# k2-fsa/Flow2GAN

Hardware: AMD Instinct MI355X
Metric: audio-seconds/sec (train step, G+D fwd/bwd) mel_24k_base (higher is better)
Workload: dtype f32 (fp32-class products on the bf16 matrix pipe for the long reductions and the direct MRD convs: every fp32 operand as three bf16 pieces = 24 significand bits, the six v_mfma_f32_32x32x16_bf16 products with i + j <= 2 per fp32 product, fp32 accumulate, error <= 2^-23 per product; short reductions ; 1 GPU; mel_24k_base GAN stage-2 train step: D-step + G-step, each on its own batch (MPD+MRD+FM+multi-scale mel), fwd+bwd+grad all-reduce, no optimizer (metric is fwd/bwd); per_gpu_batch=64, gan=gan_multi_scale_mel_recon, parallelism=dp1, optimizer=none

## Files before the change

### flow2gan_amd/csrc/conv32x6.hip

```cpp
#include <stdlib.h>

#include "common.h"


namespace {

typedef float f32x16 __attribute__((ext_vector_type(16)));
typedef float f32x4 __attribute__((ext_vector_type(4)));
typedef __bf16 bf16x8 __attribute__((ext_vector_type(8)));
typedef unsigned int u32x2 __attribute__((ext_vector_type(2)));
typedef unsigned int u32x4 __attribute__((ext_vector_type(4)));

constexpr int C = 32, KH = 3, KW = 9, NTAP = KH * KW;
constexpr int PB = 208;
constexpr int TG = 4;
constexpr int WBB = C * PB;
constexpr int WCH = C * 12;

__device__ __attribute__((aligned(16))) float c6_zero[4] = {0.f, 0.f, 0.f, 0.f};

__device__ __forceinline__ void split3(const f32x4 v, u32x2& p0, u32x2& p1, u32x2& p2) {
  unsigned a0, a1, a2, b0, b1, b2;
  f2g_split3_pair(v.x, v.y, a0, a1, a2);
  f2g_split3_pair(v.z, v.w, b0, b1, b2);
  p0 = u32x2{a0, b0};
  p1 = u32x2{a1, b1};
  p2 = u32x2{a2, b2};
}

__device__ __forceinline__ void store_px3(unsigned char* p, const f32x4 v) {
  u32x2 p0, p1, p2;
  split3(v, p0, p1, p2);
  *reinterpret_cast<u32x2*>(p) = p0;
  *reinterpret_cast<u32x2*>(p + 64) = p1;
  *reinterpret_cast<u32x2*>(p + 128) = p2;
}

struct frag6 {
  bf16x8 v[2][3];
};
__device__ __forceinline__ void ld6(frag6& f, const unsigned char* p) {
#pragma unroll
  for (int ks = 0; ks < 2; ++ks)
#pragma unroll
    for (int q = 0; q < 3; ++q) f.v[ks][q] = *reinterpret_cast<const bf16x8*>(p + q * 64 + ks * 32);
}
__device__ __forceinline__ void mm6(const frag6& a, const frag6& b, f32x16& acc0, f32x16& acc1) {
#define F2G_X6_PAIR(I, J)                                                               \
  acc0 = __builtin_amdgcn_mfma_f32_32x32x16_bf16(a.v[0][I], b.v[0][J], acc0, 0, 0, 0);   \
  acc1 = __builtin_amdgcn_mfma_f32_32x32x16_bf16(a.v[1][I], b.v[1][J], acc1, 0, 0, 0);
  F2G_X6_PAIR(2, 0) F2G_X6_PAIR(1, 1) F2G_X6_PAIR(0, 2) F2G_X6_PAIR(1, 0) F2G_X6_PAIR(0, 1) F2G_X6_PAIR(0, 0)
#undef F2G_X6_PAIR
}
__device__ __forceinline__ void tap6(const unsigned char* Ab, const unsigned char* Bb, f32x16& acc0, f32x16& acc1) {
  frag6 a, b;
  ld6(a, Ab);
  ld6(b, Bb);
  mm6(a, b, acc0, acc1);
}

template <int D>
__device__ __forceinline__ int div_small(int x) {
  static_assert(D == 39 || D == 23 || D == 20 || D == 12, "magic constants below");
  return (x * (D == 39 ? 1681 : D == 23 ? 2850 : D == 20 ? 3277 : 5462)) >> 16;
}

template <int TW_>
__device__ __forceinline__ void px_of_row(int pg, int r, int& ph, int& pw) {
  if (TW_ == 16) {
    ph = 2 * pg + (r >> 4);
    pw = (r + 12 * (r >> 4)) & 15;
  } else {
    const int p = pg * 32 + r;
    ph = p / TW_;
    pw = p % TW_;
  }
}

struct wplan {
  int src[3];
  int dst[3];
  int u[3];
};

template <int TH_, int TW_>
__global__ __launch_bounds__(512, 1) void conv32_s2_fwd6_kernel(const f2g_conv32_desc d, int tiles_w,
                                                               int tiles_h, int ntiles) {
  constexpr int IHv = TH_ + KH - 1, IWv = TW_ + (KW - 1) / 2, XW = 2 * IWv - 1;
  constexpr int SUBB = IHv * IWv * PB + 64;
  constexpr int NCHK = (IHv * XW * (C / 4) + 511) / 512;
  constexpr int NG = (NTAP + TG - 1) / TG + 1;
  static_assert(NG % 2 == 0, "the weight double buffer must come back to buffer 0 at a tile's end");
  static_assert(TH_ * TW_ == 128, "a block owns 128 output pixels");
  extern __shared__ __attribute__((aligned(16))) unsigned char smb[];
  unsigned char* At = smb;
  unsigned char* Bt = smb + 2 * SUBB;
  float* red = reinterpret_cast<float*>(Bt + 2 * TG * WBB);
  const int tid = threadIdx.x, lane = tid & 63, wave = tid >> 6;
  const int li = lane & 31, hh = lane >> 5;
  const int pg = wave & 3, half = wave >> 2;
  const int c4 = tid & 7;
  const int px0 = tid >> 3;
  auto tile_pos = [&](int tile, int& sq, int& h0, int& w0) {
    const int tw = tile % tiles_w, rest = tile / tiles_w;
    const int th = rest % tiles_h;
    sq = rest / tiles_h;
    h0 = th * TH_;
    w0 = tw * TW_;
  };
  auto load_patch = [&](int tile, f32x4 (&pf)[NCHK]) {
    int sq, h0, w0;
    tile_pos(tile, sq, h0, w0);
    const int x0 = 2 * w0 - (KW - 1) / 2;
    const float* org = d.x + (long long)sq * d.x_seq + (long long)(h0 - 1) * d.x_line + (long long)x0 * C + c4 * 4;
#pragma unroll
    for (int q = 0; q < NCHK; ++q) {
      const int px = px0 + 64 * q;
      const int r = div_small<XW>(px), xr = px - r * XW;
      const int h = h0 - 1 + r, x = x0 + xr;
      const bool ok = px < IHv * XW && h >= 0 && h < d.H && x >= 0 && x < d.Win;
      pf[q] = *reinterpret_cast<const f32x4*>(ok ? org + (long long)r * d.x_line + xr * C : c6_zero);
    }
  };
  auto store_patch = [&](const f32x4 (&pf)[NCHK]) {
// ... 53 lines not shown
    f32x16 acc0, acc1;
#pragma unroll
    for (int e = 0; e < 16; ++e) { acc0[e] = 0.f; acc1[e] = 0.f; }
#pragma unroll
    for (int g = 0; g < NG; ++g) {
      load_w(g + 1 < NG ? g + 1 : 0, wn);
      const int buf = g & 1;
#pragma unroll
      for (int u2 = 0; u2 < 2; ++u2) {
        const int t0 = g * TG + u2, t1 = g * TG + 2 + u2;
        if (t0 < NTAP && (half ? t1 : t0) < NTAP)
          tap6(Ap + (half ? F2G_C6_AOFF(t1) : F2G_C6_AOFF(t0)), Bp + (buf * TG + half * 2 + u2) * WBB, acc0, acc1);
      }
      store_w(buf ^ 1, wn);
      __syncthreads();
    }
#undef F2G_C6_AOFF
#pragma unroll
    for (int e = 0; e < 16; ++e) acc0[e] += acc1[e];
    if (half == 1) {
#pragma unroll
      for (int e = 0; e < 16; ++e) red[(pg * 16 + e) * 64 + lane] = acc0[e];
    }
    if (more) store_patch(pf);
    __syncthreads();
    if (half == 0) {
      int sq, h0, w0;
      tile_pos(tile, sq, h0, w0);
      float* ys = d.y + (long long)sq * d.y_seq;
      float* turn = red + pg * (16 * 64);
      float v[16];
#pragma unroll
      for (int e = 0; e < 16; ++e) {
        v[e] = acc0[e] + red[(pg * 16 + e) * 64 + lane] + bias;
        if (d.lrelu_slope != 0.f) v[e] = v[e] > 0.f ? v[e] : d.lrelu_slope * v[e];
      }
      __builtin_amdgcn_wave_barrier();
#pragma unroll
      for (int e = 0; e < 16; ++e) turn[((e & 3) + 8 * (e >> 2) + 4 * hh) * 32 + li] = v[e];
      __builtin_amdgcn_wave_barrier();
#pragma unroll
      for (int j = 0; j < 4; ++j) {
        int qh, qw;
        px_of_row<TW_>(pg, (lane >> 3) + 8 * j, qh, qw);
        const int oh = h0 + qh, ow = w0 + qw;
        const f32x4 u = *reinterpret_cast<const f32x4*>(turn + ((lane >> 3) + 8 * j) * 32 + 4 * (lane & 7));
        if (oh < d.H && ow < d.Wout)
          *reinterpret_cast<f32x4*>(ys + (long long)oh * d.y_line + (long long)ow * C + 4 * (lane & 7)) = u;
      }
    }
  }
}

template <int TH_, int TW_>
__global__ __launch_bounds__(512, 1) void conv32_s2_dgrad6_kernel(const f2g_conv32_desc d, int tiles_w,
                                                                 int tiles_h, int ntiles) {
  constexpr int IHv = TH_ + KH - 1, GWv = TW_ + 4;
  constexpr int NCHK = (IHv * GWv * (C / 4) + 511) / 512;
  constexpr int NG = 8;
  static_assert(TH_ * TW_ == 128, "a block owns 128 positions of each column parity");
  extern __shared__ __attribute__((aligned(16))) unsigned char smb[];
  unsigned char* At = smb;
  unsigned char* Bt = smb + IHv * GWv * PB;
  float* turn = reinterpret_cast<float*>(Bt + 2 * TG * WBB) + (threadIdx.x >> 6) * (32 * 32);
  const int tid = threadIdx.x, lane = tid & 63, wave = tid >> 6;
  const int li = lane & 31, hh = lane >> 5;
  const int pg = wave & 3, E = wave >> 2;
  const int c4 = tid & 7;
  const int NU = E ? 4 : 5, NT = KH * NU;
  const int Wp = (d.Win + 1 - E) / 2;
  const int px0 = tid >> 3;
  auto tile_pos = [&](int tile, int& sq, int& h0, int& m0) {
    const int tw = tile % tiles_w, rest = tile / tiles_w;
    const int th = rest % tiles_h;
    sq = rest / tiles_h;
    h0 = th * TH_;
    m0 = tw * TW_;
  };
  auto load_patch = [&](int tile, f32x4 (&pf)[NCHK]) {
    int sq, h0, m0;
    tile_pos(tile, sq, h0, m0);
    const float* org = d.x + (long long)sq * d.x_seq + (long long)(h0 - 1) * d.x_line + (long long)(m0 - 2) * C + c4 * 4;
#pragma unroll
    for (int q = 0; q < NCHK; ++q) {
      const int px = px0 + 64 * q;
      const int r = div_small<GWv>(px), xc = px - r * GWv;
      const int h = h0 - 1 + r, c = m0 - 2 + xc;
      const bool ok = px < IHv * GWv && h >= 0 && h < d.H && c >= 0 && c < d.Wout;
      pf[q] = *reinterpret_cast<const f32x4*>(ok ? org + (long long)r * d.x_line + xc * C : c6_zero);
    }
  };
  auto store_patch = [&](const f32x4 (&pf)[NCHK]) {
#pragma unroll
    for (int q = 0; q < NCHK; ++q) {
      const int px = px0 + 64 * q;
      if (px < IHv * GWv) store_px3(At + px * PB + c4 * 8, pf[q]);
    }
  };
  const unsigned char* wimg = reinterpret_cast<const unsigned char*>(d.w);
  int wsrc[3], wdst[3], wslot[3];
#pragma unroll
  for (int k = 0; k < 3; ++k) {
    const int c = tid + 512 * k;
    const int u = c / WCH, rem = c - u * WCH;
    const int row = rem / 12, part = rem - row * 12;
    wslot[k] = u;
    wsrc[k] = row * 192 + part * 16;
    wdst[k] = u * WBB + row * PB + part * 16;
  }
  auto load_w = [&](int g, u32x4 (&wn)[3]) {
#pragma unroll
    for (int k = 0; k < 3; ++k) {
      const int e = wslot[k] >> 1, nu = e ? 4 : 5, nt = KH * nu;
      int ti = 2 * g + (wslot[k] & 1);
      ti = ti < nt ? ti : nt - 1;
      const int dh = e ? ti >> 2 : (ti * 13) >> 6;
      const int tile_w = dh * KW + e + 2 * (ti - dh * nu);
      wn[k] = *reinterpret_cast<const u32x4*>(wimg + (long long)tile_w * (C * 192) + wsrc[k]);
    }
  };
  auto store_w = [&](int buf, const u32x4 (&wn)[3]) {
#pragma unroll
    for (int k = 0; k < 3; ++k) *reinterpret_cast<u32x4*>(Bt + buf * (TG * WBB) + wdst[k]) = wn[k];
  };
  int ph, pw;
  px_of_row<TW_>(pg, li, ph, pw);
  const unsigned char* Ap = At + ((ph + 2) * GWv + pw + 4) * PB + hh * 16;
  const unsigned char* Bp = Bt + (E * 2) * WBB + li * PB + hh * 16;
  const bool msk = d.mask_src != nullptr, fm = d.fm_ref != nullptr;
  const float fmw = fm ? d.fm_w * (d.fm_wdev ? d.fm_wdev[0] : 1.f) : 0.f;
  float cs[4] = {0.f, 0.f, 0.f, 0.f};

  int tile = blockIdx.x;
  if (tile >= ntiles) return;
  u32x4 wn[3];
  {
    f32x4 pf[NCHK];
    load_patch(tile, pf);
    load_w(0, wn);
    store_patch(pf);
    store_w(0, wn);
  }
  __syncthreads();
  for (; tile < ntiles; tile += gridDim.x) {
    const int nxt = tile + gridDim.x;
    const bool more = nxt < ntiles;
    f32x4 pf[NCHK];
    load_patch(more ? nxt : tile, pf);
    int sq, h0, m0;
    tile_pos(tile, sq, h0, m0);
    long long ioff[4];
    f32x4 my[4];
#pragma unroll
    for (int j = 0; j < 4; ++j) {
      int qh, qw;
      px_of_row<TW_>(pg, (lane >> 3) + 8 * j, qh, qw);
      const int oh = h0 + qh, om = m0 + qw;
      ioff[j] = (oh < d.H && om < Wp)
                    ? (long long)sq * d.y_seq + (long long)oh * d.y_line + (long long)(2 * om + E) * C + 4 * (lane & 7)
                    : -1;
      if (msk && !fm) my[j] = *reinterpret_cast<const f32x4*>(d.mask_src + (ioff[j] >= 0 ? ioff[j] : 0));
    }
    f32x16 acc0, acc1;
#pragma unroll
    for (int e = 0; e < 16; ++e) { acc0[e] = 0.f; acc1[e] = 0.f; }
#define F2G_C6_GOFF(TI) ((E ? ((TI) / 4) * GWv + (TI) % 4 : ((TI) / 5) * GWv + (TI) % 5) * PB)
#pragma unroll
    for (int g = 0; g < NG; ++g) {
      load_w(g + 1 < NG ? g + 1 : 0, wn);
      const int buf = g & 1;
#pragma unroll
      for (int u2 = 0; u2 < 2; ++u2)
        if (2 * g + u2 < NT) tap6(Ap - F2G_C6_GOFF(2 * g + u2), Bp + (buf * TG + u2) * WBB, acc0, acc1);
      store_w(buf ^ 1, wn);
      __syncthreads();
    }
#undef F2G_C6_GOFF
#pragma unroll
    for (int q = 0; q < 16; ++q) turn[((q & 3) + 8 * (q >> 2) + 4 * hh) * 32 + li] = acc0[q] + acc1[q];
    __builtin_amdgcn_wave_barrier();
    auto item = [&](int j) {
      return *reinterpret_cast<const f32x4*>(turn + ((lane >> 3) + 8 * j) * 32 + 4 * (lane & 7));
    };
    if (!msk) {
#pragma unroll
      for (int j = 0; j < 4; ++j) {
        const f32x4 u = item(j);
        if (ioff[j] < 0) continue;
        cs[0] += u.x, cs[1] += u.y, cs[2] += u.z, cs[3] += u.w;
        *reinterpret_cast<f32x4*>(d.y + ioff[j]) = u;
      }
    } else if (!fm) {
#pragma unroll
      for (int j = 0; j < 4; ++j) {
        const f32x4 u = item(j);
        if (ioff[j] < 0) continue;
        f32x4 v;
        v.x = u.x * (my[j].x > 0.f ? 1.f : d.mask_slope);
        v.y = u.y * (my[j].y > 0.f ? 1.f : d.mask_slope);
        v.z = u.z * (my[j].z > 0.f ? 1.f : d.mask_slope);
        v.w = u.w * (my[j].w > 0.f ? 1.f : d.mask_slope);
        cs[0] += v.x, cs[1] += v.y, cs[2] += v.z, cs[3] += v.w;
        *reinterpret_cast<f32x4*>(d.y + ioff[j]) = v;
      }
    } else {
      f32x4 yv[4], fv[4];
#pragma unroll
      for (int j = 0; j < 4; ++j) {
        const long long o = ioff[j] >= 0 ? ioff[j] : 0;
        yv[j] = *reinterpret_cast<const f32x4*>(d.mask_src + o);
        fv[j] = *reinterpret_cast<const f32x4*>(d.fm_ref + o);
      }
#pragma unroll
      for (int j = 0; j < 4; ++j) {
        const f32x4 u = item(j);
        if (ioff[j] < 0) continue;
        float v[4] = {u.x, u.y, u.z, u.w};
        const float y[4] = {yv[j].x, yv[j].y, yv[j].z, yv[j].w}, f[4] = {fv[j].x, fv[j].y, fv[j].z, fv[j].w};
#pragma unroll
        for (int e = 0; e < 4; ++e) {
          const float dl = y[e] - f[e];
          v[e] += fmw * (dl > 0.f ? 1.f : (dl < 0.f ? -1.f : 0.f));
          v[e] *= y[e] > 0.f ? 1.f : d.mask_slope;
          cs[e] += v[e];
        }
        *reinterpret_cast<f32x4*>(d.y + ioff[j]) = f32x4{v[0], v[1], v[2], v[3]};
      }
    }
    __builtin_amdgcn_wave_barrier();
    if (more) store_patch(pf);
    __syncthreads();
  }
  if (d.colsum) {
#pragma unroll
    for (int e = 0; e < 4; ++e) {
      float v = cs[e];
      v += __shfl_xor(v, 8);
      v += __shfl_xor(v, 16);
      v += __shfl_xor(v, 32);
      if (lane < 8) atomicAdd(d.colsum + 4 * lane + e, v);
    }
  }
}

template <int TH_, int TW_>
__global__ __launch_bounds__(512, 1) void conv32_s2_dgrad6m_kernel(const f2g_conv32_desc d, int tiles_w,
                                                                 int tiles_h, int ntiles) {
  constexpr int IHv = TH_ + KH - 1, GWv = TW_ + 4;
  constexpr int NCHK = (IHv * GWv * (C / 4) + 511) / 512;
  constexpr int NG = 8;
  static_assert(TH_ * TW_ == 128, "a block owns 128 positions of each column parity");
  extern __shared__ __attribute__((aligned(16))) unsigned char smb[];
  unsigned char* At = smb;
  unsigned char* Bt = smb + IHv * GWv * PB;
  const int tid = threadIdx.x, lane = tid & 63, wave = tid >> 6;
  const int li = lane & 31, hh = lane >> 5;
  const int pg = wave & 3, E = wave >> 2;
  const int c4 = tid & 7;
  const int NU = E ? 4 : 5, NT = KH * NU;
  const int Wp = (d.Win + 1 - E) / 2;
  const int px0 = tid >> 3;
  auto tile_pos = [&](int tile, int& sq, int& h0, int& m0) {
    const int tw = tile % tiles_w, rest = tile / tiles_w;
    const int th = rest % tiles_h;
    sq = rest / tiles_h;
    h0 = th * TH_;
    m0 = tw * TW_;
  };
  auto load_patch = [&](int tile, f32x4 (&pf)[NCHK]) {
    int sq, h0, m0;
    tile_pos(tile, sq, h0, m0);
    const float* org = d.x + (long long)sq * d.x_seq + (long long)(h0 - 1) * d.x_line + (long long)(m0 - 2) * C + c4 * 4;
#pragma unroll
    for (int q = 0; q < NCHK; ++q) {
      const int px = px0 + 64 * q;
      const int r = div_small<GWv>(px), xc = px - r * GWv;
      const int h = h0 - 1 + r, c = m0 - 2 + xc;
      const bool ok = px < IHv * GWv && h >= 0 && h < d.H && c >= 0 && c < d.Wout;
      pf[q] = *reinterpret_cast<const f32x4*>(ok ? org + (long long)r * d.x_line + xc * C : c6_zero);
    }
  };
  auto store_patch = [&](const f32x4 (&pf)[NCHK]) {
#pragma unroll
    for (int q = 0; q < NCHK; ++q) {
      const int px = px0 + 64 * q;
      if (px < IHv * GWv) store_px3(At + px * PB + c4 * 8, pf[q]);
    }
  };
  const unsigned char* wimg = reinterpret_cast<const unsigned char*>(d.w);
  int wsrc[3], wdst[3], wslot[3];
#pragma unroll
  for (int k = 0; k < 3; ++k) {
    const int c = tid + 512 * k;
    const int u = c / WCH, rem = c - u * WCH;
    const int row = rem / 12, part = rem - row * 12;
    wslot[k] = u;
    wsrc[k] = row * 192 + part * 16;
    wdst[k] = u * WBB + row * PB + part * 16;
  }
  auto load_w = [&](int g, u32x4 (&wn)[3]) {
#pragma unroll
    for (int k = 0; k < 3; ++k) {
      const int e = wslot[k] >> 1, nu = e ? 4 : 5, nt = KH * nu;
      int ti = 2 * g + (wslot[k] & 1);
      ti = ti < nt ? ti : nt - 1;
      const int dh = e ? ti >> 2 : (ti * 13) >> 6;
      const int tile_w = dh * KW + e + 2 * (ti - dh * nu);
      wn[k] = *reinterpret_cast<const u32x4*>(wimg + (long long)tile_w * (C * 192) + wsrc[k]);
    }
  };
  auto store_w = [&](int buf, const u32x4 (&wn)[3]) {
#pragma unroll
    for (int k = 0; k < 3; ++k) *reinterpret_cast<u32x4*>(Bt + buf * (TG * WBB) + wdst[k]) = wn[k];
  };
  int ph, pw;
  px_of_row<TW_>(pg, li, ph, pw);
  const unsigned char* Ap = At + ((ph + 2) * GWv + pw + 4) * PB + hh * 16;
  const unsigned char* Bp = Bt + (E * 2) * WBB + li * PB + hh * 16;
  const bool msk = d.mask_src != nullptr, fm = d.fm_ref != nullptr;
  const float fmw = fm ? d.fm_w * (d.fm_wdev ? d.fm_wdev[0] : 1.f) : 0.f;
  float cs = 0.f;

  int tile = blockIdx.x;
  if (tile >= ntiles) return;
  u32x4 wn[3];
  {
    f32x4 pf[NCHK];
    load_patch(tile, pf);
    load_w(0, wn);
    store_patch(pf);
    store_w(0, wn);
  }
  __syncthreads();
  for (; tile < ntiles; tile += gridDim.x) {
    const int nxt = tile + gridDim.x;
    const bool more = nxt < ntiles;
    f32x4 pf[NCHK];
    load_patch(more ? nxt : tile, pf);
    int sq, h0, m0;
    tile_pos(tile, sq, h0, m0);
    float my[16];
    if (msk && !fm) {
#pragma unroll
      for (int q = 0; q < 16; ++q) {
        int qh, qw;
        px_of_row<TW_>(pg, (q & 3) + 8 * (q >> 2) + 4 * hh, qh, qw);
        const int oh = h0 + qh, om = m0 + qw;
        const long long off = (long long)sq * d.y_seq + (long long)oh * d.y_line + (long long)(2 * om + E) * C + li;
        my[q] = (oh < d.H && om < Wp) ? d.mask_src[off] : 1.f;
      }
    }
    f32x16 acc0, acc1;
#pragma unroll
    for (int e = 0; e < 16; ++e) { acc0[e] = 0.f; acc1[e] = 0.f; }
#define F2G_C6_GOFF(TI) ((E ? ((TI) / 4) * GWv + (TI) % 4 : ((TI) / 5) * GWv + (TI) % 5) * PB)
#pragma unroll
    for (int g = 0; g < NG; ++g) {
      load_w(g + 1 < NG ? g + 1 : 0, wn);
      const int buf = g & 1;
#pragma unroll
      for (int u2 = 0; u2 < 2; ++u2)
        if (2 * g + u2 < NT) tap6(Ap - F2G_C6_GOFF(2 * g + u2), Bp + (buf * TG + u2) * WBB, acc0, acc1);
      store_w(buf ^ 1, wn);
      __syncthreads();
    }
#undef F2G_C6_GOFF
#pragma unroll
    for (int q = 0; q < 16; ++q) {
      int qh, qw;
      px_of_row<TW_>(pg, (q & 3) + 8 * (q >> 2) + 4 * hh, qh, qw);
      const int oh = h0 + qh, om = m0 + qw;
      if (oh < d.H && om < Wp) {
        const long long off = (long long)sq * d.y_seq + (long long)oh * d.y_line + (long long)(2 * om + E) * C + li;
        float v = acc0[q] + acc1[q];
        if (msk) {
          const float y = fm ? d.mask_src[off] : my[q];
          if (fm) {
            const float dl = y - d.fm_ref[off];
            v += fmw * (dl > 0.f ? 1.f : (dl < 0.f ? -1.f : 0.f));
          }
          v *= y > 0.f ? 1.f : d.mask_slope;
        }
        cs += v;
        d.y[off] = v;
      }
    }
    if (more) store_patch(pf);
    __syncthreads();
  }
  if (d.colsum) {
    cs += __shfl_xor(cs, 32);
    if (hh == 0) atomicAdd(d.colsum + li, cs);
  }
}

typedef short s16x4 __attribute__((ext_vector_type(4)));
constexpr int GPL = 128 * 64;
constexpr int GCH = 128 * (C / 4) / 512;

__device__ __forceinline__ bf16x8 tr_pix8(const unsigned char* p) {
  typedef s16x4 __attribute__((address_space(3))) * lds_p;
  const s16x4 a = __builtin_amdgcn_ds_read_tr16_b64_v4i16((lds_p)(p));
  const s16x4 b = __builtin_amdgcn_ds_read_tr16_b64_v4i16((lds_p)(p + 4 * 64));
  return __builtin_bit_cast(bf16x8, __builtin_shufflevector(a, b, 0, 1, 2, 3, 4, 5, 6, 7));
}

template <int TH, int TW>
__global__ __launch_bounds__(512, 1) void conv32_s2_wgrad6_kernel(const f2g_conv32_desc d, float* gw,
                                                                  int tiles_h, int tiles_w,
                                                                  int tiles_per_block) {
  constexpr int IH = TH + KH - 1, IW = TW + (KW - 1) / 2, XW = 2 * IW - 1;
  constexpr int XPAR = IH * IW * 64 + 64;
  constexpr int XPL = 2 * XPAR;
  constexpr int XCH = (IH * XW * (C / 4) + 511) / 512;
  constexpr int KR = 16 / TW;
  constexpr int NK = TH / KR;
  static_assert(TH * TW == 128 && NK == 8 && XCH <= NK && GCH <= NK, "tile shapes");
  extern __shared__ __attribute__((aligned(16))) unsigned char smb[];
  unsigned char* Xp = smb;
  unsigned char* Gp = smb + 3 * XPL;
  const int tid = threadIdx.x, lane = tid & 63, wave = tid >> 6;
  const int li = lane & 31, hh = lane >> 5;
  const int ntiles = d.S * tiles_h * tiles_w;
  f32x16 acc[6];
#pragma unroll
  for (int a = 0; a < 6; ++a)
#pragma unroll
    for (int e = 0; e < 16; ++e) acc[a][e] = 0.f;
  const int g4 = lane >> 4, i16 = lane & 15;
  const int kpix = (g4 >> 1) * 8 + (i16 >> 2);
  const int kpat = TW == 16 ? kpix : (g4 >> 1) * IW + (i16 >> 2);
  const int chb = (g4 & 1) * 32 + (i16 & 3) * 8;
  int xo[3], xs[3];
#pragma unroll
  for (int a = 0; a < 3; ++a) {
    int t = wave + 8 * a;
    int dh = t / KW, j = t - dh * KW;
    xo[a] = (j & 1) * XPAR + (dh * IW + (j >> 1) + kpat) * 64 + chb;
    t = 24 + a;
    dh = t / KW;
    j = t - dh * KW;
    xs[a] = (j & 1) * XPAR + (dh * IW + (j >> 1) + kpat) * 64 + chb;
  }
  const int go = kpix * 64 + chb;
  const int c4 = tid & 7, px0 = tid >> 3;
// ... 321 lines not shown
    for (int q = 0; q < NQ; ++q) {
      const int px = (tid + 512 * q) >> 3;
      u32x2 pk[3];
      if (xrow[q] > -(1 << 21)) {
        split3(px_[q], pk[0], pk[1], pk[2]);
#pragma unroll
        for (int pc = 0; pc < 3; ++pc) *reinterpret_cast<u32x2*>(Xp + pc * W33_XPL + (px + 1) * 64 + c4 * 8) = pk[pc];
      }
      if (grow[q] > -(1 << 21)) {
        split3(pg_[q], pk[0], pk[1], pk[2]);
#pragma unroll
        for (int pc = 0; pc < 3; ++pc) *reinterpret_cast<u32x2*>(Gp + pc * W33_GPL + px * 64 + c4 * 8) = pk[pc];
      }
    }
    __syncthreads();
    for (int ks = wave; ks < nks; ks += 8) {
      bf16x8 a[3];
#pragma unroll
      for (int q = 0; q < 3; ++q) a[q] = tr_pix8(Gp + q * W33_GPL + ks * (16 * 64) + go);
#pragma unroll
      for (int t = 0; t < T33; ++t) {
        bf16x8 b[3];
#pragma unroll
        for (int q = 0; q < 3; ++q) b[q] = tr_pix8(Xp + q * W33_XPL + ks * (16 * 64) + xo[t]);
        mfma6(a, b, acc[t]);
      }
    }
    __syncthreads();
  }
  float* red = reinterpret_cast<float*>(smb);
#pragma unroll
  for (int t = 0; t < T33; ++t) {
    __syncthreads();
#pragma unroll
    for (int e = 0; e < 16; ++e) red[(wave * 16 + e) * 64 + lane] = acc[t][e];
    __syncthreads();
    if (wave == (t & 7)) {
#pragma unroll
      for (int e = 0; e < 16; ++e) {
        float v = 0.f;
#pragma unroll
        for (int w8 = 0; w8 < 8; ++w8) v += red[(w8 * 16 + e) * 64 + lane];
        const int co = (e & 3) + 8 * (e >> 2) + 4 * hh;
        atomicAdd(gw + co * (T33 * C) + t * C + li, v);
      }
    }
  }
}

template <int TH_, int TW_>
constexpr size_t fwd6_smem() {
  return (size_t)2 * ((TH_ + 2) * (TW_ + 4) * PB + 64) + 2 * TG * WBB + 4 * 16 * 64 * sizeof(float);
}
template <int TH_, int TW_>
constexpr size_t dgrad6_smem() {
  return (size_t)(TH_ + 2) * (TW_ + 4) * PB + 2 * TG * WBB + 8 * 32 * 32 * sizeof(float);
}

}

int f2g_conv32_fwd6_launch(const f2g_conv32_desc* d, hipStream_t st) {
  auto waste = [&](int th, int tw) {
    return (long long)((d->H + th - 1) / th * th) * ((d->Wout + tw - 1) / tw * tw);
  };
  const bool tall = waste(16, 8) < waste(8, 16);
  const int th = tall ? 16 : 8, tw = tall ? 8 : 16;
  const int tiles_h = (d->H + th - 1) / th, tiles_w = (d->Wout + tw - 1) / tw;
  const long long nt = (long long)tiles_h * tiles_w * d->S;
  if (nt >= (1ll << 30) || d->x_line >= (1ll << 24)) return F2G_EINVAL;
  static bool attr = false;
  if (!attr) {
    (void)hipFuncSetAttribute(reinterpret_cast<const void*>(conv32_s2_fwd6_kernel<8, 16>),
                              hipFuncAttributeMaxDynamicSharedMemorySize, (int)(fwd6_smem<8, 16>()));
    (void)hipFuncSetAttribute(reinterpret_cast<const void*>(conv32_s2_fwd6_kernel<16, 8>),
                              hipFuncAttributeMaxDynamicSharedMemorySize, (int)(fwd6_smem<16, 8>()));
    attr = true;
  }
  const int grid = (int)(nt < 256 ? nt : 256);
  if (tall)
    hipLaunchKernelGGL((conv32_s2_fwd6_kernel<16, 8>), dim3(grid), dim3(512), (fwd6_smem<16, 8>()), st, *d,
                       tiles_w, tiles_h, (int)nt);
  else
    hipLaunchKernelGGL((conv32_s2_fwd6_kernel<8, 16>), dim3(grid), dim3(512), (fwd6_smem<8, 16>()), st, *d,
                       tiles_w, tiles_h, (int)nt);
  return f2g_check_launch();
}

int f2g_conv32_dgrad6_launch(const f2g_conv32_desc* d, hipStream_t st) {
  const int Wp0 = (d->Win + 1) / 2;
  auto waste = [&](int th, int tw) {
    return (long long)((d->H + th - 1) / th * th) * ((Wp0 + tw - 1) / tw * tw);
  };
  const bool tall = waste(16, 8) < waste(8, 16);
  const int th = tall ? 16 : 8, tw = tall ? 8 : 16;
  const int tiles_h = (d->H + th - 1) / th, tiles_w = (Wp0 + tw - 1) / tw;
  const long long nt = (long long)tiles_h * tiles_w * d->S;
  if (nt >= (1ll << 30) || d->x_line >= (1ll << 24)) return F2G_EINVAL;
  static bool attr = false;
  if (!attr) {
    (void)hipFuncSetAttribute(reinterpret_cast<const void*>(conv32_s2_dgrad6_kernel<8, 16>),
                              hipFuncAttributeMaxDynamicSharedMemorySize, (int)(dgrad6_smem<8, 16>()));
    (void)hipFuncSetAttribute(reinterpret_cast<const void*>(conv32_s2_dgrad6_kernel<16, 8>),
                              hipFuncAttributeMaxDynamicSharedMemorySize, (int)(dgrad6_smem<16, 8>()));
    attr = true;
  }
  const int grid = (int)(nt < 256 ? nt : 256);
  if (d->mask_src) {
    static bool attrm = false;
    if (!attrm) {
      (void)hipFuncSetAttribute(reinterpret_cast<const void*>(conv32_s2_dgrad6m_kernel<8, 16>),
                                hipFuncAttributeMaxDynamicSharedMemorySize, (int)(dgrad6_smem<8, 16>()));
      (void)hipFuncSetAttribute(reinterpret_cast<const void*>(conv32_s2_dgrad6m_kernel<16, 8>),
                                hipFuncAttributeMaxDynamicSharedMemorySize, (int)(dgrad6_smem<16, 8>()));
      attrm = true;
    }
    if (tall)
      hipLaunchKernelGGL((conv32_s2_dgrad6m_kernel<16, 8>), dim3(grid), dim3(512), (dgrad6_smem<16, 8>()), st, *d,
                         tiles_w, tiles_h, (int)nt);
    else
      hipLaunchKernelGGL((conv32_s2_dgrad6m_kernel<8, 16>), dim3(grid), dim3(512), (dgrad6_smem<8, 16>()), st, *d,
                         tiles_w, tiles_h, (int)nt);
    return f2g_check_launch();
  }
  if (tall)
    hipLaunchKernelGGL((conv32_s2_dgrad6_kernel<16, 8>), dim3(grid), dim3(512), (dgrad6_smem<16, 8>()), st, *d,
                       tiles_w, tiles_h, (int)nt);
  else
    hipLaunchKernelGGL((conv32_s2_dgrad6_kernel<8, 16>), dim3(grid), dim3(512), (dgrad6_smem<8, 16>()), st, *d,
                       tiles_w, tiles_h, (int)nt);
  return f2g_check_launch();
}

int f2g_conv32_wgrad6_launch(const f2g_conv32_desc* d, float* gw, hipStream_t st) {
  auto waste = [&](int th, int tw) {
    return (long long)((d->H + th - 1) / th * th) * ((d->Wout + tw - 1) / tw * tw);
  };
  const bool tall = waste(16, 8) < waste(8, 16);
  const int th = tall ? 16 : 8, tw = tall ? 8 : 16;
  const int tiles_h = (d->H + th - 1) / th, tiles_w = (d->Wout + tw - 1) / tw;
  const long long nt = (long long)d->S * tiles_h * tiles_w;
  if (nt >= (1ll << 30) || d->x_line >= (1ll << 24)) return F2G_EINVAL;
  int per = (int)((nt + 255) / 256);
  if (per < 1) per = 1;
  constexpr size_t sm8 = (size_t)3 * 2 * ((8 + 2) * (16 + 4) * 64 + 64) + 3 * GPL;
  constexpr size_t sm16 = (size_t)3 * 2 * ((16 + 2) * (8 + 4) * 64 + 64) + 3 * GPL;
  static_assert(sm8 >= (size_t)8 * 16 * 64 * 4 && sm16 >= (size_t)8 * 16 * 64 * 4,
                "the flush reuses the planes as its reduction buffer");
  static bool attr = false;
  if (!attr) {
    (void)hipFuncSetAttribute(reinterpret_cast<const void*>(conv32_s2_wgrad6_kernel<8, 16>),
                              hipFuncAttributeMaxDynamicSharedMemorySize, (int)sm8);
    (void)hipFuncSetAttribute(reinterpret_cast<const void*>(conv32_s2_wgrad6_kernel<16, 8>),
                              hipFuncAttributeMaxDynamicSharedMemorySize, (int)sm16);
    attr = true;
  }
  const unsigned grid = (unsigned)((nt + per - 1) / per);
  if (tall)
    hipLaunchKernelGGL((conv32_s2_wgrad6_kernel<16, 8>), dim3(grid), dim3(512), sm16, st, *d, gw, tiles_h, tiles_w, per);
  else
    hipLaunchKernelGGL((conv32_s2_wgrad6_kernel<8, 16>), dim3(grid), dim3(512), sm8, st, *d, gw, tiles_h, tiles_w, per);
  return f2g_check_launch();
}

extern "C" int f2g_conv33_fwd(const f2g_conv32_desc* d, f2g_stream_t stream) {
  if (!d || !d->x || !d->w || !d->y || d->precision != 3 || d->Win != d->Wout || d->fm_ref) return F2G_EINVAL;
  if ((((uintptr_t)d->x) & 15) || (((uintptr_t)d->w) & 15) || (d->x_line & 3) || (d->x_seq & 3)) return F2G_EINVAL;
  if (d->S <= 0 || d->H <= 0 || d->Win <= 0) return F2G_OK;
  const int W = d->Win;
  if (W > 112 || d->x_line >= (1ll << 24)) return F2G_EINVAL;
  if (d->y_line < (long long)W * C || (d->y != d->x && d->y_seq < (long long)d->H * d->y_line)) return F2G_EINVAL;
  if ((d->y_line & 3) || (d->y_seq & 3) || (((uintptr_t)d->y) & 15)) return F2G_EINVAL;
  if (d->mask_src && (d->lrelu_slope != 0.f || d->bias || (((uintptr_t)d->mask_src) & 15))) {
    f2g_set_error("f2g_conv33_fwd: mask_src (data-gradient role) excludes bias / lrelu_slope (forward role)");
    return F2G_EINVAL;
  }
  int R = 256 / W;
  if (R > d->H) R = d->H;
  while (R > 1 && (R + 2) * (W + 2) > P33) --R;
  if (R < 1 || (R + 2) * (W + 2) > P33) return F2G_EINVAL;
  const int tiles_h = (d->H + R - 1) / R;
  const long long nt = (long long)tiles_h * d->S;
  if (nt >= (1ll << 30)) return F2G_EINVAL;
// ... 44 lines not shown
```

Before: 804.1 audio-s/s.

## Restructure stride-2 conv dgrad so each wave computes both output parities

The dgrad kernel is reorganised so every wave owns both even and odd output columns of a 256-position tile, instead of splitting waves by parity. Each A fragment loaded from LDS now feeds two MFMA chains (even and odd weights) through an interleaved mm6x2, and the tap schedule is regrouped into 7 groups with one special group for the odd-only last tap. The masked and unmasked variants merge into a single template; the masked path keeps values in registers and prefetches mask bits instead of using the LDS transpose. Tile shapes grow to 16x16, 8x32 or 32x8. The intent is to cut A-fragment LDS traffic and barrier count per output, at the cost of more registers and smaller grids for small inputs.

Result: no change. 807.6 audio-s/s (median of 4 runs) (+0.4%).

```diff
diff --git a/flow2gan_amd/csrc/conv32x6.hip b/flow2gan_amd/csrc/conv32x6.hip
--- a/flow2gan_amd/csrc/conv32x6.hip
+++ b/flow2gan_amd/csrc/conv32x6.hip
@@ -52,6 +52,16 @@
   F2G_X6_PAIR(2, 0) F2G_X6_PAIR(1, 1) F2G_X6_PAIR(0, 2) F2G_X6_PAIR(1, 0) F2G_X6_PAIR(0, 1) F2G_X6_PAIR(0, 0)
 #undef F2G_X6_PAIR
 }
+__device__ __forceinline__ void mm6x2(const frag6& a0, const frag6& b0, const frag6& a1, const frag6& b1, f32x16& c0,
+                                      f32x16& c1) {
+#define F2G_X6_PAIR2(I, J)                                                          \
+  c0 = __builtin_amdgcn_mfma_f32_32x32x16_bf16(a0.v[0][I], b0.v[0][J], c0, 0, 0, 0); \
+  c1 = __builtin_amdgcn_mfma_f32_32x32x16_bf16(a1.v[0][I], b1.v[0][J], c1, 0, 0, 0); \
+  c0 = __builtin_amdgcn_mfma_f32_32x32x16_bf16(a0.v[1][I], b0.v[1][J], c0, 0, 0, 0); \
+  c1 = __builtin_amdgcn_mfma_f32_32x32x16_bf16(a1.v[1][I], b1.v[1][J], c1, 0, 0, 0);
+  F2G_X6_PAIR2(2, 0) F2G_X6_PAIR2(1, 1) F2G_X6_PAIR2(0, 2) F2G_X6_PAIR2(1, 0) F2G_X6_PAIR2(0, 1) F2G_X6_PAIR2(0, 0)
+#undef F2G_X6_PAIR2
+}
 __device__ __forceinline__ void tap6(const unsigned char* Ab, const unsigned char* Bb, f32x16& acc0, f32x16& acc1) {
   frag6 a, b;
   ld6(a, Ab);
@@ -61,8 +71,8 @@
 
 template <int D>
 __device__ __forceinline__ int div_small(int x) {
-  static_assert(D == 39 || D == 23 || D == 20 || D == 12, "magic constants below");
-  return (x * (D == 39 ? 1681 : D == 23 ? 2850 : D == 20 ? 3277 : 5462)) >> 16;
+  static_assert(D == 39 || D == 23 || D == 36 || D == 20 || D == 12, "magic constants below");
+  return (x * (D == 39 ? 1681 : D == 23 ? 2850 : D == 36 ? 1821 : D == 20 ? 3277 : 5462)) >> 16;
 }
 
 template <int TW_>
@@ -70,6 +80,10 @@
   if (TW_ == 16) {
     ph = 2 * pg + (r >> 4);
     pw = (r + 12 * (r >> 4)) & 15;
+  } else if (TW_ == 8) {
+    const int j = r >> 3;
+    ph = 4 * pg + j;
+    pw = (r + 4 * ((j ^ (j >> 1)) & 1)) & 7;
   } else {
     const int p = pg * 32 + r;
     ph = p / TW_;
@@ -229,23 +243,22 @@
   }
 }
 
-template <int TH_, int TW_>
+constexpr int DG_NG = 7;
+constexpr int DG_TURN = 16 * 32 * 4;
+
+template <int TH_, int TW_, bool MASKED>
 __global__ __launch_bounds__(512, 1) void conv32_s2_dgrad6_kernel(const f2g_conv32_desc d, int tiles_w,
                                                                  int tiles_h, int ntiles) {
   constexpr int IHv = TH_ + KH - 1, GWv = TW_ + 4;
   constexpr int NCHK = (IHv * GWv * (C / 4) + 511) / 512;
-  constexpr int NG = 8;
-  static_assert(TH_ * TW_ == 128, "a block owns 128 positions of each column parity");
+  static_assert(TH_ * TW_ == 256, "a block owns 256 positions of each column parity");
   extern __shared__ __attribute__((aligned(16))) unsigned char smb[];
   unsigned char* At = smb;
   unsigned char* Bt = smb + IHv * GWv * PB;
-  float* turn = reinterpret_cast<float*>(Bt + 2 * TG * WBB) + (threadIdx.x >> 6) * (32 * 32);
-  const int tid = threadIdx.x, lane = tid & 63, wave = tid >> 6;
+  const int tid = threadIdx.x, lane = tid & 63, pg = tid >> 6;
   const int li = lane & 31, hh = lane >> 5;
-  const int pg = wave & 3, E = wave >> 2;
   const int c4 = tid & 7;
-  const int NU = E ? 4 : 5, NT = KH * NU;
-  const int Wp = (d.Win + 1 - E) / 2;
+  const int Wp0 = (d.Win + 1) / 2, Wp1 = d.Win / 2;
   const int px0 = tid >> 3;
   auto tile_pos = [&](int tile, int& sq, int& h0, int& m0) {
     const int tw = tile % tiles_w, rest = tile / tiles_w;
@@ -257,14 +270,15 @@
   auto load_patch = [&](int tile, f32x4 (&pf)[NCHK]) {
     int sq, h0, m0;
     tile_pos(tile, sq, h0, m0);
-    const float* org = d.x + (long long)sq * d.x_seq + (long long)(h0 - 1) * d.x_line + (long long)(m0 - 2) * C + c4 * 4;
+    const float* org = d.x + (long long)sq * d.x_seq + (long long)(h0 - 1) * d.x_line + (long long)(m0 - 2) * C;
 #pragma unroll
     for (int q = 0; q < NCHK; ++q) {
       const int px = px0 + 64 * q;
       const int r = div_small<GWv>(px), xc = px - r * GWv;
       const int h = h0 - 1 + r, c = m0 - 2 + xc;
       const bool ok = px < IHv * GWv && h >= 0 && h < d.H && c >= 0 && c < d.Wout;
-      pf[q] = *reinterpret_cast<const f32x4*>(ok ? org + (long long)r * d.x_line + xc * C : c6_zero);
+      const unsigned o = (unsigned)r * (unsigned)d.x_line + (unsigned)(xc * C + c4 * 4);
+      pf[q] = *reinterpret_cast<const f32x4*>(ok ? org + o : c6_zero);
     }
   };
   auto store_patch = [&](const f32x4 (&pf)[NCHK]) {
@@ -288,12 +302,15 @@
   auto load_w = [&](int g, u32x4 (&wn)[3]) {
 #pragma unroll
     for (int k = 0; k < 3; ++k) {
-      const int e = wslot[k] >> 1, nu = e ? 4 : 5, nt = KH * nu;
-      int ti = 2 * g + (wslot[k] & 1);
-      ti = ti < nt ? ti : nt - 1;
-      const int dh = e ? ti >> 2 : (ti * 13) >> 6;
-      const int tile_w = dh * KW + e + 2 * (ti - dh * nu);
-      wn[k] = *reinterpret_cast<const u32x4*>(wimg + (long long)tile_w * (C * 192) + wsrc[k]);
+      const int s = wslot[k];
+      int tap;
+      if (g < DG_NG - 1) {
+        const int p = 2 * g + (s >> 1);
+        tap = (p >> 2) * KW + 2 * (p & 3) + (s & 1);
+      } else {
+        tap = (s < KH ? s : KH - 1) * KW + KW - 1;
+      }
+      wn[k] = *reinterpret_cast<const u32x4*>(wimg + tap * (C * 192) + wsrc[k]);
     }
   };
   auto store_w = [&](int buf, const u32x4 (&wn)[3]) {
@@ -303,14 +320,15 @@
   int ph, pw;
   px_of_row<TW_>(pg, li, ph, pw);
   const unsigned char* Ap = At + ((ph + 2) * GWv + pw + 4) * PB + hh * 16;
-  const unsigned char* Bp = Bt + (E * 2) * WBB + li * PB + hh * 16;
-  const bool msk = d.mask_src != nullptr, fm = d.fm_ref != nullptr;
+  const unsigned char* Bp = Bt + li * PB + hh * 16;
+  const bool fm = MASKED && d.fm_ref != nullptr;
   const float fmw = fm ? d.fm_w * (d.fm_wdev ? d.fm_wdev[0] : 1.f) : 0.f;
   float cs[4] = {0.f, 0.f, 0.f, 0.f};
 
   int tile = blockIdx.x;
   if (tile >= ntiles) return;
   u32x4 wn[3];
+  int cur = 0;
   {
     f32x4 pf[NCHK];
     load_patch(tile, pf);
@@ -326,248 +344,139 @@
     load_patch(more ? nxt : tile, pf);
     int sq, h0, m0;
     tile_pos(tile, sq, h0, m0);
-    long long ioff[4];
-    f32x4 my[4];
-#pragma unroll
-    for (int j = 0; j < 4; ++j) {
+    const long long ybase = (long long)sq * d.y_seq + (long long)h0 * d.y_line + (long long)(2 * m0) * C;
+    float* const ys = d.y + ybase;
+    auto out_off = [&](int r, int e, int ch) {
       int qh, qw;
-      px_of_row<TW_>(pg, (lane >> 3) + 8 * j, qh, qw);
-      const int oh = h0 + qh, om = m0 + qw;
-      ioff[j] = (oh < d.H && om < Wp)
-                    ? (long long)sq * d.y_seq + (long long)oh * d.y_line + (long long)(2 * om + E) * C + 4 * (lane & 7)
-                    : -1;
-      if (msk && !fm) my[j] = *reinterpret_cast<const f32x4*>(d.mask_src + (ioff[j] >= 0 ? ioff[j] : 0));
-    }
-    f32x16 acc0, acc1;
-#pragma unroll
-    for (int e = 0; e < 16; ++e) { acc0[e] = 0.f; acc1[e] = 0.f; }
-#define F2G_C6_GOFF(TI) ((E ? ((TI) / 4) * GWv + (TI) % 4 : ((TI) / 5) * GWv + (TI) % 5) * PB)
-#pragma unroll
-    for (int g = 0; g < NG; ++g) {
-      load_w(g + 1 < NG ? g + 1 : 0, wn);
-      const int buf = g & 1;
-#pragma unroll
-      for (int u2 = 0; u2 < 2; ++u2)
-        if (2 * g + u2 < NT) tap6(Ap - F2G_C6_GOFF(2 * g + u2), Bp + (buf * TG + u2) * WBB, acc0, acc1);
-      store_w(buf ^ 1, wn);
+      px_of_row<TW_>(pg, r, qh, qw);
+      return (h0 + qh < d.H && m0 + qw < (e ? Wp1 : Wp0)) ? qh * (int)d.y_line + (2 * qw + e) * C + ch : -1;
+    };
+    float mt[16];
+    unsigned mbits = 0u;
+    auto quad_off = [&](int qb, int& nv0, int& nv1) {
+      int qh, qw;
+      px_of_row<TW_>(pg, 8 * qb + 4 * hh, qh, qw);
+      const bool rowok = h0 + qh < d.H;
+      nv0 = rowok ? Wp0 - (m0 + qw) : 0;
+      nv1 = rowok ? Wp1 - (m0 + qw) : 0;
+      return qh * (int)d.y_line + 2 * qw * C + li;
+    };
+    auto mask_request = [&](int e) {
+#pragma unroll
+      for (int qb = 0; qb < 4; ++qb) {
+        int nv0, nv1;
+        const float* mp = d.mask_src + ybase + quad_off(qb, nv0, nv1);
+#pragma unroll
+        for (int qi = 0; qi < 4; ++qi) mt[4 * qb + qi] = qi < (e ? nv1 : nv0) ? mp[(2 * qi + e) * C] : 1.f;
+      }
+    };
+    auto mask_fold = [&](int e) {
+#pragma unroll
+      for (int q = 0; q < 16; ++q) mbits |= (mt[q] > 0.f ? 1u : 0u) << (16 * e + q);
+    };
+    f32x16 acc[2];
+#pragma unroll
+    for (int e = 0; e < 16; ++e) { acc[0][e] = 0.f; acc[1][e] = 0.f; }
+#pragma unroll
+    for (int g = 0; g < DG_NG; ++g) {
+      load_w(g + 1 < DG_NG ? g + 1 : 0, wn);
+      if (MASKED && !fm) {
+        if (g == 2 || g == 4) mask_fold(g / 2 - 1);
+        if (g == 0 || g == 2) mask_request(g / 2);
+      }
+      const unsigned char* Bc = Bp + cur * (TG * WBB);
+      if (g < DG_NG - 1) {
+#pragma unroll
+        for (int u2 = 0; u2 < 2; ++u2) {
+          const int p = 2 * g + u2;
+          frag6 a, be, bo;
+          ld6(a, Ap - ((p >> 2) * GWv + (p & 3)) * PB);
+          ld6(be, Bc + (2 * u2) * WBB);
+          ld6(bo, Bc + (2 * u2 + 1) * WBB);
+          mm6x2(a, be, a, bo, acc[0], acc[1]);
+          __builtin_amdgcn_sched_barrier(0);
+        }
+      } else {
+        f32x16 t;
+#pragma unroll
+        for (int e = 0; e < 16; ++e) t[e] = 0.f;
+#pragma unroll
+        for (int dh = 0; dh < KH; ++dh) {
+          tap6(Ap - (dh * GWv + 4) * PB, Bc + dh * WBB, acc[0], t);
+          __builtin_amdgcn_sched_barrier(0);
+        }
+#pragma unroll
+        for (int e = 0; e < 16; ++e) acc[0][e] += t[e];
+      }
+      cur ^= 1;
+      store_w(cur, wn);
       __syncthreads();
     }
-#undef F2G_C6_GOFF
-#pragma unroll
-    for (int q = 0; q < 16; ++q) turn[((q & 3) + 8 * (q >> 2) + 4 * hh) * 32 + li] = acc0[q] + acc1[q];
-    __builtin_amdgcn_wave_barrier();
-    auto item = [&](int j) {
-      return *reinterpret_cast<const f32x4*>(turn + ((lane >> 3) + 8 * j) * 32 + 4 * (lane & 7));
-    };
-    if (!msk) {
-#pragma unroll
-      for (int j = 0; j < 4; ++j) {
-        const f32x4 u = item(j);
-        if (ioff[j] < 0) continue;
-        cs[0] += u.x, cs[1] += u.y, cs[2] += u.z, cs[3] += u.w;
-        *reinterpret_cast<f32x4*>(d.y + ioff[j]) = u;
-      }
-    } else if (!fm) {
-#pragma unroll
-      for (int j = 0; j < 4; ++j) {
-        const f32x4 u = item(j);
-        if (ioff[j] < 0) continue;
-        f32x4 v;
-        v.x = u.x * (my[j].x > 0.f ? 1.f : d.mask_slope);
-        v.y = u.y * (my[j].y > 0.f ? 1.f : d.mask_slope);
-        v.z = u.z * (my[j].z > 0.f ? 1.f : d.mask_slope);
-        v.w = u.w * (my[j].w > 0.f ? 1.f : d.mask_slope);
-        cs[0] += v.x, cs[1] += v.y, cs[2] += v.z, cs[3] += v.w;
-        *reinterpret_cast<f32x4*>(d.y + ioff[j]) = v;
+    if (MASKED) {
+#pragma unroll
+      for (int qb = 0; qb < 4; ++qb) {
+        int nv[2];
+        const long long qo = ybase + quad_off(qb, nv[0], nv[1]);
+        float* const yq = d.y + qo;
+        const float* const mq = d.mask_src + qo;
+        const float* const fq = d.fm_ref + qo;
+#pragma unroll
+        for (int e = 0; e < 2; ++e)
+#pragma unroll
+          for (int qi = 0; qi < 4; ++qi) {
+            if (qi >= nv[e]) continue;
+            const int q = 4 * qb + qi, off = (2 * qi + e) * C;
+            float v = acc[e][q];
+            bool pos = (mbits >> (16 * e + q)) & 1u;
+            if (fm) {
+              const float y = mq[off], dl = y - fq[off];
+              v += fmw * (dl > 0.f ? 1.f : (dl < 0.f ? -1.f : 0.f));
+              pos = y > 0.f;
+            }
+            v *= pos ? 1.f : d.mask_slope;
+            cs[0] += v;
+            yq[off] = v;
+          }
       }
     } else {
-      f32x4 yv[4], fv[4];
-#pragma unroll
-      for (int j = 0; j < 4; ++j) {
-        const long long o = ioff[j] >= 0 ? ioff[j] : 0;
-        yv[j] = *reinterpret_cast<const f32x4*>(d.mask_src + o);
-        fv[j] = *reinterpret_cast<const f32x4*>(d.fm_ref + o);
-      }
-#pragma unroll
-      for (int j = 0; j < 4; ++j) {
-        const f32x4 u = item(j);
-        if (ioff[j] < 0) continue;
-        float v[4] = {u.x, u.y, u.z, u.w};
-        const float y[4] = {yv[j].x, yv[j].y, yv[j].z, yv[j].w}, f[4] = {fv[j].x, fv[j].y, fv[j].z, fv[j].w};
-#pragma unroll
-        for (int e = 0; e < 4; ++e) {
-          const float dl = y[e] - f[e];
-          v[e] += fmw * (dl > 0.f ? 1.f : (dl < 0.f ? -1.f : 0.f));
-          v[e] *= y[e] > 0.f ? 1.f : d.mask_slope;
-          cs[e] += v[e];
+      float* turn = reinterpret_cast<float*>(Bt + 2 * TG * WBB + pg * DG_TURN);
+#pragma unroll
+      for (int e = 0; e < 2; ++e)
+#pragma unroll
+        for (int half = 0; half < 2; ++half) {
+#pragma unroll
+          for (int q = 0; q < 8; ++q) turn[((q & 3) + 8 * (q >> 2) + 4 * hh) * 32 + li] = acc[e][8 * half + q];
+          __builtin_amdgcn_wave_barrier();
+#pragma unroll
+          for (int j = 0; j < 2; ++j) {
+            const int pos = (lane >> 3) + 8 * j;
+            const f32x4 u = *reinterpret_cast<const f32x4*>(turn + pos * 32 + 4 * (lane & 7));
+            const int off = out_off(16 * half + pos, e, 4 * (lane & 7));
+            if (off < 0) continue;
+            cs[0] += u.x, cs[1] += u.y, cs[2] += u.z, cs[3] += u.w;
+            *reinterpret_cast<f32x4*>(ys + off) = u;
+          }
+          __builtin_amdgcn_wave_barrier();
         }
-        *reinterpret_cast<f32x4*>(d.y + ioff[j]) = f32x4{v[0], v[1], v[2], v[3]};
-      }
-    }
-    __builtin_amdgcn_wave_barrier();
+    }
     if (more) store_patch(pf);
     __syncthreads();
   }
   if (d.colsum) {
-#pragma unroll
-    for (int e = 0; e < 4; ++e) {
-      float v = cs[e];
-      v += __shfl_xor(v, 8);
-      v += __shfl_xor(v, 16);
+    if (MASKED) {
+      float v = cs[0];
       v += __shfl_xor(v, 32);
-      if (lane < 8) atomicAdd(d.colsum + 4 * lane + e, v);
-    }
-  }
-}
-
-template <int TH_, int TW_>
-__global__ __launch_bounds__(512, 1) void conv32_s2_dgrad6m_kernel(const f2g_conv32_desc d, int tiles_w,
-                                                                 int tiles_h, int ntiles) {
-  constexpr int IHv = TH_ + KH - 1, GWv = TW_ + 4;
-  constexpr int NCHK = (IHv * GWv * (C / 4) + 511) / 512;
-  constexpr int NG = 8;
-  static_assert(TH_ * TW_ == 128, "a block owns 128 positions of each column parity");
-  extern __shared__ __attribute__((aligned(16))) unsigned char smb[];
-  unsigned char* At = smb;
-  unsigned char* Bt = smb + IHv * GWv * PB;
-  const int tid = threadIdx.x, lane = tid & 63, wave = tid >> 6;
-  const int li = lane & 31, hh = lane >> 5;
-  const int pg = wave & 3, E = wave >> 2;
-  const int c4 = tid & 7;
-  const int NU = E ? 4 : 5, NT = KH * NU;
-  const int Wp = (d.Win + 1 - E) / 2;
-  const int px0 = tid >> 3;
-  auto tile_pos = [&](int tile, int& sq, int& h0, int& m0) {
-    const int tw = tile % tiles_w, rest = tile / tiles_w;
-    const int th = rest % tiles_h;
-    sq = rest / tiles_h;
-    h0 = th * TH_;
-    m0 = tw * TW_;
-  };
-  auto load_patch = [&](int tile, f32x4 (&pf)[NCHK]) {
-    int sq, h0, m0;
-    tile_pos(tile, sq, h0, m0);
-    const float* org = d.x + (long long)sq * d.x_seq + (long long)(h0 - 1) * d.x_line + (long long)(m0 - 2) * C + c4 * 4;
-#pragma unroll
-    for (int q = 0; q < NCHK; ++q) {
-      const int px = px0 + 64 * q;
-      const int r = div_small<GWv>(px), xc = px - r * GWv;
-      const int h = h0 - 1 + r, c = m0 - 2 + xc;
-      const bool ok = px < IHv * GWv && h >= 0 && h < d.H && c >= 0 && c < d.Wout;
-      pf[q] = *reinterpret_cast<const f32x4*>(ok ? org + (long long)r * d.x_line + xc * C : c6_zero);
-    }
-  };
-  auto store_patch = [&](const f32x4 (&pf)[NCHK]) {
-#pragma unroll
-    for (int q = 0; q < NCHK; ++q) {
-      const int px = px0 + 64 * q;
-      if (px < IHv * GWv) store_px3(At + px * PB + c4 * 8, pf[q]);
-    }
-  };
-  const unsigned char* wimg = reinterpret_cast<const unsigned char*>(d.w);
-  int wsrc[3], wdst[3], wslot[3];
-#pragma unroll
-  for (int k = 0; k < 3; ++k) {
-    const int c = tid + 512 * k;
-    const int u = c / WCH, rem = c - u * WCH;
-    const int row = rem / 12, part = rem - row * 12;
-    wslot[k] = u;
-    wsrc[k] = row * 192 + part * 16;
-    wdst[k] = u * WBB + row * PB + part * 16;
-  }
-  auto load_w = [&](int g, u32x4 (&wn)[3]) {
-#pragma unroll
-    for (int k = 0; k < 3; ++k) {
-      const int e = wslot[k] >> 1, nu = e ? 4 : 5, nt = KH * nu;
-      int ti = 2 * g + (wslot[k] & 1);
-      ti = ti < nt ? ti : nt - 1;
-      const int dh = e ? ti >> 2 : (ti * 13) >> 6;
-      const int tile_w = dh * KW + e + 2 * (ti - dh * nu);
-      wn[k] = *reinterpret_cast<const u32x4*>(wimg + (long long)tile_w * (C * 192) + wsrc[k]);
-    }
-  };
-  auto store_w = [&](int buf, const u32x4 (&wn)[3]) {
-#pragma unroll
-    for (int k = 0; k < 3; ++k) *reinterpret_cast<u32x4*>(Bt + buf * (TG * WBB) + wdst[k]) = wn[k];
-  };
-  int ph, pw;
-  px_of_row<TW_>(pg, li, ph, pw);
-  const unsigned char* Ap = At + ((ph + 2) * GWv + pw + 4) * PB + hh * 16;
-  const unsigned char* Bp = Bt + (E * 2) * WBB + li * PB + hh * 16;
-  const bool msk = d.mask_src != nullptr, fm = d.fm_ref != nullptr;
-  const float fmw = fm ? d.fm_w * (d.fm_wdev ? d.fm_wdev[0] : 1.f) : 0.f;
-  float cs = 0.f;
-
-  int tile = blockIdx.x;
-  if (tile >= ntiles) return;
-  u32x4 wn[3];
-  {
-    f32x4 pf[NCHK];
-    load_patch(tile, pf);
-    load_w(0, wn);
-    store_patch(pf);
-    store_w(0, wn);
-  }
-  __syncthreads();
-  for (; tile < ntiles; tile += gridDim.x) {
-    const int nxt = tile + gridDim.x;
-    const bool more = nxt < ntiles;
-    f32x4 pf[NCHK];
-    load_patch(more ? nxt : tile, pf);
-    int sq, h0, m0;
-    tile_pos(tile, sq, h0, m0);
-    float my[16];
-    if (msk && !fm) {
-#pragma unroll
-      for (int q = 0; q < 16; ++q) {
-        int qh, qw;
-        px_of_row<TW_>(pg, (q & 3) + 8 * (q >> 2) + 4 * hh, qh, qw);
-        const int oh = h0 + qh, om = m0 + qw;
-        const long long off = (long long)sq * d.y_seq + (long long)oh * d.y_line + (long long)(2 * om + E) * C + li;
-        my[q] = (oh < d.H && om < Wp) ? d.mask_src[off] : 1.f;
-      }
-    }
-    f32x16 acc0, acc1;
-#pragma unroll
-    for (int e = 0; e < 16; ++e) { acc0[e] = 0.f; acc1[e] = 0.f; }
-#define F2G_C6_GOFF(TI) ((E ? ((TI) / 4) * GWv + (TI) % 4 : ((TI) / 5) * GWv + (TI) % 5) * PB)
-#pragma unroll
-    for (int g = 0; g < NG; ++g) {
-      load_w(g + 1 < NG ? g + 1 : 0, wn);
-      const int buf = g & 1;
-#pragma unroll
-      for (int u2 = 0; u2 < 2; ++u2)
-        if (2 * g + u2 < NT) tap6(Ap - F2G_C6_GOFF(2 * g + u2), Bp + (buf * TG + u2) * WBB, acc0, acc1);
-      store_w(buf ^ 1, wn);
-      __syncthreads();
-    }
-#undef F2G_C6_GOFF
-#pragma unroll
-    for (int q = 0; q < 16; ++q) {
-      int qh, qw;
-      px_of_row<TW_>(pg, (q & 3) + 8 * (q >> 2) + 4 * hh, qh, qw);
-      const int oh = h0 + qh, om = m0 + qw;
-      if (oh < d.H && om < Wp) {
-        const long long off = (long long)sq * d.y_seq + (long long)oh * d.y_line + (long long)(2 * om + E) * C + li;
-        float v = acc0[q] + acc1[q];
-        if (msk) {
-          const float y = fm ? d.mask_src[off] : my[q];
-          if (fm) {
-            const float dl = y - d.fm_ref[off];
-            v += fmw * (dl > 0.f ? 1.f : (dl < 0.f ? -1.f : 0.f));
-          }
-          v *= y > 0.f ? 1.f : d.mask_slope;
-        }
-        cs += v;
-        d.y[off] = v;
-      }
-    }
-    if (more) store_patch(pf);
-    __syncthreads();
-  }
-  if (d.colsum) {
-    cs += __shfl_xor(cs, 32);
-    if (hh == 0) atomicAdd(d.colsum + li, cs);
+      if (hh == 0) atomicAdd(d.colsum + li, v);
+    } else {
+#pragma unroll
+      for (int e = 0; e < 4; ++e) {
+        float v = cs[e];
+        v += __shfl_xor(v, 8);
+        v += __shfl_xor(v, 16);
+        v += __shfl_xor(v, 32);
+        if (lane < 8) atomicAdd(d.colsum + 4 * lane + e, v);
+      }
+    }
   }
 }
 
@@ -995,9 +904,9 @@
 constexpr size_t fwd6_smem() {
   return (size_t)2 * ((TH_ + 2) * (TW_ + 4) * PB + 64) + 2 * TG * WBB + 4 * 16 * 64 * sizeof(float);
 }
-template <int TH_, int TW_>
+template <int TH_, int TW_, bool MASKED>
 constexpr size_t dgrad6_smem() {
-  return (size_t)(TH_ + 2) * (TW_ + 4) * PB + 2 * TG * WBB + 8 * 32 * 32 * sizeof(float);
+  return (size_t)(TH_ + 2) * (TW_ + 4) * PB + 2 * TG * WBB + (MASKED ? 0 : 8 * DG_TURN);
 }
 
 }
@@ -1029,48 +938,37 @@
   return f2g_check_launch();
 }
 
+template <int TH_, int TW_, bool MASKED>
+static void dgrad6_run(const f2g_conv32_desc* d, int Wp0, hipStream_t st) {
+  constexpr size_t smem = dgrad6_smem<TH_, TW_, MASKED>();
+  static_assert(smem <= 160 * 1024, "one block per CU");
+  static bool attr = false;
+  if (!attr) {
+    (void)hipFuncSetAttribute(reinterpret_cast<const void*>(conv32_s2_dgrad6_kernel<TH_, TW_, MASKED>),
+                              hipFuncAttributeMaxDynamicSharedMemorySize, (int)smem);
+    attr = true;
+  }
+  const int tiles_h = (d->H + TH_ - 1) / TH_, tiles_w = (Wp0 + TW_ - 1) / TW_;
+  const long long nt = (long long)tiles_h * tiles_w * d->S;
+  const int grid = (int)(nt < 256 ? nt : 256);
+  hipLaunchKernelGGL((conv32_s2_dgrad6_kernel<TH_, TW_, MASKED>), dim3(grid), dim3(512), smem, st, *d, tiles_w,
+                     tiles_h, (int)nt);
+}
+
 int f2g_conv32_dgrad6_launch(const f2g_conv32_desc* d, hipStream_t st) {
   const int Wp0 = (d->Win + 1) / 2;
   auto waste = [&](int th, int tw) {
     return (long long)((d->H + th - 1) / th * th) * ((Wp0 + tw - 1) / tw * tw);
   };
-  const bool tall = waste(16, 8) < waste(8, 16);
-  const int th = tall ? 16 : 8, tw = tall ? 8 : 16;
-  const int tiles_h = (d->H + th - 1) / th, tiles_w = (Wp0 + tw - 1) / tw;
-  const long long nt = (long long)tiles_h * tiles_w * d->S;
-  if (nt >= (1ll << 30) || d->x_line >= (1ll << 24)) return F2G_EINVAL;
-  static bool attr = false;
-  if (!attr) {
-    (void)hipFuncSetAttribute(reinterpret_cast<const void*>(conv32_s2_dgrad6_kernel<8, 16>),
-                              hipFuncAttributeMaxDynamicSharedMemorySize, (int)(dgrad6_smem<8, 16>()));
-    (void)hipFuncSetAttribute(reinterpret_cast<const void*>(conv32_s2_dgrad6_kernel<16, 8>),
-                              hipFuncAttributeMaxDynamicSharedMemorySize, (int)(dgrad6_smem<16, 8>()));
-    attr = true;
-  }
-  const int grid = (int)(nt < 256 ? nt : 256);
-  if (d->mask_src) {
-    static bool attrm = false;
-    if (!attrm) {
-      (void)hipFuncSetAttribute(reinterpret_cast<const void*>(conv32_s2_dgrad6m_kernel<8, 16>),
-                                hipFuncAttributeMaxDynamicSharedMemorySize, (int)(dgrad6_smem<8, 16>()));
-      (void)hipFuncSetAttribute(reinterpret_cast<const void*>(conv32_s2_dgrad6m_kernel<16, 8>),
-                                hipFuncAttributeMaxDynamicSharedMemorySize, (int)(dgrad6_smem<16, 8>()));
-      attrm = true;
-    }
-    if (tall)
-      hipLaunchKernelGGL((conv32_s2_dgrad6m_kernel<16, 8>), dim3(grid), dim3(512), (dgrad6_smem<16, 8>()), st, *d,
-                         tiles_w, tiles_h, (int)nt);
-    else
-      hipLaunchKernelGGL((conv32_s2_dgrad6m_kernel<8, 16>), dim3(grid), dim3(512), (dgrad6_smem<8, 16>()), st, *d,
-                         tiles_w, tiles_h, (int)nt);
-    return f2g_check_launch();
-  }
-  if (tall)
-    hipLaunchKernelGGL((conv32_s2_dgrad6_kernel<16, 8>), dim3(grid), dim3(512), (dgrad6_smem<16, 8>()), st, *d,
-                       tiles_w, tiles_h, (int)nt);
-  else
-    hipLaunchKernelGGL((conv32_s2_dgrad6_kernel<8, 16>), dim3(grid), dim3(512), (dgrad6_smem<8, 16>()), st, *d,
-                       tiles_w, tiles_h, (int)nt);
+  int shape = 0;
+  long long best = waste(16, 16);
+  if (waste(8, 32) < best) shape = 1, best = waste(8, 32);
+  if (waste(32, 8) < best) shape = 2, best = waste(32, 8);
+  if (best / 256 * d->S >= (1ll << 30) || d->x_line >= (1ll << 24) || d->y_line >= (1ll << 24)) return F2G_EINVAL;
+  const bool m = d->mask_src != nullptr;
+  if (shape == 0) m ? dgrad6_run<16, 16, true>(d, Wp0, st) : dgrad6_run<16, 16, false>(d, Wp0, st);
+  else if (shape == 1) m ? dgrad6_run<8, 32, true>(d, Wp0, st) : dgrad6_run<8, 32, false>(d, Wp0, st);
+  else m ? dgrad6_run<32, 8, true>(d, Wp0, st) : dgrad6_run<32, 8, false>(d, Wp0, st);
   return f2g_check_launch();
 }
 
```
